# coop-columb/two-tower-amazon-recommender

Hardware: AMD Instinct MI355X
Metric: user-item pairs/sec (train step) + embedding-gather HBM GB/s, 1/2/4/8 MI355X (higher is better)
Workload: dtype f32; 1 GPU; cfg3: 5000000 users x 10000000 items, emb_dim 128, towers 128->256->128, batch 8192, in-batch sampled softmax T=0.1, sgd lr 1e-3, ids U; global_batch=8192, parallelism=single GPU

## Files before the change

### two_tower_amazon_recommender_amd/csrc/score.hip

```cpp
#include "common.h"

namespace {

using tt::f32x4;
using tt::f32x16;
typedef __bf16 bf16x4 __attribute__((ext_vector_type(4)));
typedef __bf16 bf16x8 __attribute__((ext_vector_type(8)));
typedef short s16x4 __attribute__((ext_vector_type(4)));

constexpr float kLog2e = 1.44269504088896340736f;
constexpr float kLn2 = 0.69314718055994530942f;
constexpr float kNegBig = -1.0e30f;

enum { MODE_FWD = 0, MODE_BWD = 1, MODE_FUSED = 2, MODE_RANK = 3, MODE_FUSED_S = 4, MODE_BWD_S = 5 };
constexpr float kRescaleThr = 8.0f;

struct ScoreArgs {
  const float* R;
  const float* K;
  int64_t n_r, n_c;
  int64_t diag;
  float c1;
  const float* a_r;
  const float* s_r;
  const float* a_c;
  const float* s_c;
  const int64_t* id_r;
  const int64_t* id_c;
  int nsplit;
  int64_t c_per_split;
  float* part_m;
  float* part_l;
  float* pos2;
  float* slab;
  const float* h_r;
  const float* h_c;
  const int64_t* pos_idx;
  int32_t* part_cnt;
  float* S;
  int64_t ldS;
};

template <int D, int PREC>
struct Geo {
  static constexpr int LS = D + 4;
  static constexpr int NG = D / 8;
  static constexpr int NB = D / 32;
  static constexpr int KS = D / 16;
  static constexpr int HALF_B = 32 * 256;
  static constexpr int PIECE_B = (D / 128) * HALF_B;
  static constexpr int TILE_F = PREC == 0 ? 32 * LS : 3 * PIECE_B / 4;
  static constexpr int BUF_F = TILE_F + 160;
  static constexpr int LDS_BYTES = 2 * BUF_F * 4;
};

struct Bf3 {
  __bf16 hi, mid, lo;
};
__device__ __forceinline__ Bf3 split3(float x) {
  Bf3 o;
  o.hi = (__bf16)x;
  const float r1 = x - (float)o.hi;
  o.mid = (__bf16)r1;
  o.lo = (__bf16)(r1 - (float)o.mid);
  return o;
}

__device__ __forceinline__ int img_off(int row, int ch) { return 256 * row + 16 * (ch ^ (((row & 3) << 2) | ((row >> 2) & 3))); }

constexpr int kBwdSWaves = 2;
constexpr int kSPrefetch = 2;
#ifndef TT_LOOP_LAMBDA
#define TT_LOOP_LAMBDA 0
#endif
constexpr int kTilesPerBarrier = 2;
constexpr int kTilesPerBarrierBwdS = kTilesPerBarrier;
template <int D, int MODE, int PREC>
constexpr int tiles_per_barrier() {
  if (PREC == 0 && D <= 128 && MODE == MODE_BWD_S) return kTilesPerBarrierBwdS;
  return (PREC == 0 && D <= 128 && (MODE == MODE_BWD || MODE == MODE_FUSED || MODE == MODE_FUSED_S))
             ? kTilesPerBarrier : 1;
}

template <int D, int MODE, int PREC>
constexpr bool split_d() {
  return PREC == 1 && D == 256 && (MODE == MODE_BWD || MODE == MODE_FUSED || MODE == MODE_FUSED_S);
}
template <int D, int MODE, bool HAS_IDS, bool HAS_HN, int PREC>
constexpr int rf_lds_groups() {
  if (PREC == 0 && D == 256 && (MODE == MODE_FUSED || MODE == MODE_FUSED_S) && (HAS_IDS || HAS_HN))
    return (HAS_IDS && HAS_HN) ? 10 : (HAS_HN ? 8 : 5);
  if (PREC == 0 && D == 128 && MODE == MODE_BWD && HAS_IDS && HAS_HN) return 2;
  return 0;
}
template <int D, int MODE, int PREC, int WAVES>
constexpr int rows_per_wg() { return (split_d<D, MODE, PREC>() ? WAVES / 2 : WAVES) * 32; }

template <int D, int MODE, bool HAS_IDS, bool HAS_HN, int WAVES, int PREC>
__global__ __launch_bounds__(WAVES * 64, (WAVES == 8 ? 2 : (D <= 128 ? ((MODE == MODE_BWD_S && PREC == 0) ? kBwdSWaves : 2) : 1))) void score_kernel(ScoreArgs p) {
  constexpr bool IS_FUSED = MODE == MODE_FUSED || MODE == MODE_FUSED_S;
  constexpr bool IS_BWD = MODE == MODE_BWD || MODE == MODE_BWD_S;
  constexpr bool FROM_S = MODE == MODE_BWD_S, TO_S = MODE == MODE_FUSED_S;
  using G_ = Geo<D, PREC>;
  constexpr int LS = G_::LS, NG = G_::NG, NB = G_::NB, TILE_F = G_::TILE_F, BUF_F = G_::BUF_F;
  constexpr int HALF_B = G_::HALF_B, PIECE_B = G_::PIECE_B;
  constexpr bool SPLIT = split_d<D, MODE, PREC>();
  constexpr int KS = SPLIT ? G_::KS / 2 : G_::KS;
  constexpr int NBW = SPLIT ? NB / 2 : NB;
  static_assert(PREC == 0 || D % 128 == 0, "bf16x3: dim 128 / 256 only (whole [32][128] bf16 images)");
  constexpr int ROW4 = D / 4;
  constexpr int THREADS = WAVES * 64;
  constexpr int NV = (32 * ROW4 + THREADS - 1) / THREADS;
  extern __shared__ __attribute__((aligned(16))) float smem[];

  const int tid = threadIdx.x;
  const int lane = tid & 63;
  const int wave = tid >> 6;
  const int h = lane >> 5;
  const int ln = lane & 31;

  const int split = __builtin_amdgcn_readfirstlane((int)(blockIdx.x % (unsigned)p.nsplit));
  const int64_t rblk = __builtin_amdgcn_readfirstlane((int)(blockIdx.x / (unsigned)p.nsplit));
  const int hw = SPLIT ? (wave & 1) : 0;
// ... 473 lines not shown
      if constexpr (IS_BWD || IS_FUSED) {
        if constexpr (PREC == 0) { if (t + TPB < ntiles) load_tile(t + TPB); }
        if constexpr (FROM_S) { if (t + 1 < ntiles) load_S(t + 1, xs); }
        gemm2(T, coef);
      }
      if (t + TPB < ntiles) store_tile((t + TPB) % NBUF);
      if ((t % TPB) == TPB - 1) __syncthreads();
    };
    for (int t = 0; t < ntiles; t += 2) {
      tile_step(t);
      if (t + 1 < ntiles) tile_step(t + 1);
    }
#else
    for (int t = 0; t < ntiles; ++t) {
      if constexpr (MODE == MODE_FWD || MODE == MODE_RANK || PREC == 1) { if (t + 1 < ntiles) load_tile(t + 1); }
      const float* T = smem + (t % NBUF) * BUF_F;
      f32x16 X;
      if constexpr (FROM_S) X = xs; else X = gemm1(T);
      if constexpr (SPLIT) exchange(X);
      if constexpr (TO_S) store_S(t, X);
      float coef[16];
      epilogue(T, t, X, coef);
      if constexpr (IS_BWD || IS_FUSED) {
        if constexpr (PREC == 0) { if (t + TPB < ntiles) load_tile(t + TPB); }
        if constexpr (FROM_S) { if (t + 1 < ntiles) load_S(t + 1, xs); }
        gemm2(T, coef);
      }
      if (t + TPB < ntiles) store_tile((t + TPB) % NBUF);
      if ((t % TPB) == TPB - 1) __syncthreads();
    }
#endif
  }

  if constexpr (IS_FUSED) {
    const float L = run_l + __shfl_xor(run_l, 32);
    if (r_ok && hw == 0) {
      if (h == 0) {
        p.part_m[(int64_t)split * p.n_r + r] = run_m;
        p.part_l[(int64_t)split * p.n_r + r] = L;
      }
      if (have_pos) p.pos2[r] = pos;
    }
  }
  if constexpr (MODE == MODE_RANK) {
    const int total = cnt + __shfl_xor(cnt, 32);
    if (r_ok && h == 0) p.part_cnt[(int64_t)split * p.n_r + r] = total;
  } else if constexpr (MODE == MODE_FWD) {
    const float om = __shfl_xor(run_m, 32);
    const float ol = __shfl_xor(run_l, 32);
    const float M = fmaxf(run_m, om);
    const float L = run_l * __builtin_amdgcn_exp2f(run_m - M) + ol * __builtin_amdgcn_exp2f(om - M);
    if (r_ok) {
      if (h == 0) {
        p.part_m[(int64_t)split * p.n_r + r] = M;
        p.part_l[(int64_t)split * p.n_r + r] = L;
      }
      if (have_pos) p.pos2[r] = pos;
    }
  } else {
    if (r_ok) {
      float* out = p.slab + ((int64_t)split * p.n_r + r) * D + 128 * hw;
      if constexpr (PREC == 1) {
#pragma unroll
        for (int b = 0; b < NBW; ++b)
#pragma unroll
          for (int g = 0; g < 4; ++g)
            *reinterpret_cast<f32x4*>(out + 32 * b + 8 * g + 4 * h) = f32x4{G[b][4 * g], G[b][4 * g + 1], G[b][4 * g + 2], G[b][4 * g + 3]};
      } else
#pragma unroll
      for (int reg = 0; reg < 16; ++reg) {
        const int i = tt::acc_row(reg, 0) + 4 * h;
        if constexpr (NB == 8) {
          *reinterpret_cast<f32x4*>(out + 8 * i) = f32x4{G[0][reg], G[1][reg], G[2][reg], G[3][reg]};
          *reinterpret_cast<f32x4*>(out + 8 * i + 4) = f32x4{G[4][reg], G[5][reg], G[6][reg], G[7][reg]};
        } else if constexpr (NB == 4) {
          *reinterpret_cast<f32x4*>(out + 4 * i) = f32x4{G[0][reg], G[1][reg], G[2][reg], G[3][reg]};
        } else if constexpr (NB == 2) {
          *reinterpret_cast<float2*>(out + 2 * i) = float2{G[0][reg], G[1][reg]};
        } else {
          out[i] = G[0][reg];
        }
      }
    }
  }
}


__global__ __launch_bounds__(256) void prob_bias_kernel(const float* __restrict__ prob, float* __restrict__ out, int64_t n) {
  const int64_t i = (int64_t)blockIdx.x * 256 + threadIdx.x;
  if (i < n) out[i] = -__log2f(fminf(fmaxf(prob[i], 1e-6f), 1.0f));
}

__global__ __launch_bounds__(256) void bwd_prep_kernel(const float* __restrict__ lse, const float* __restrict__ w,
                                                       float* __restrict__ a, float* __restrict__ s, int64_t n,
                                                       float scale) {
  const int64_t i = (int64_t)blockIdx.x * 256 + threadIdx.x;
  if (i < n) {
    a[i] = -lse[i] * kLog2e;
    s[i] = (w != nullptr ? w[i] : 1.0f) * scale;
  }
}

__global__ __launch_bounds__(256) void fwd_combine_kernel(const float* __restrict__ part_m, const float* __restrict__ part_l,
                                                          const float* __restrict__ pos2, const float* __restrict__ w,
                                                          int64_t n_r, int nsplit, float* __restrict__ lse,
                                                          float* __restrict__ per_row) {
  const int64_t r = (int64_t)blockIdx.x * 256 + threadIdx.x;
  if (r >= n_r) return;
  float M = kNegBig;
  for (int s = 0; s < nsplit; ++s) M = fmaxf(M, part_m[(int64_t)s * n_r + r]);
  float L = 0.f;
  for (int s = 0; s < nsplit; ++s)
    L += part_l[(int64_t)s * n_r + r] * __builtin_amdgcn_exp2f(part_m[(int64_t)s * n_r + r] - M);
  const float lse2 = M + __log2f(L);
  lse[r] = lse2 * kLn2;
  per_row[r] = (lse2 - pos2[r]) * kLn2 * (w != nullptr ? w[r] : 1.0f);
}

__global__ __launch_bounds__(256) void fused_combine_kernel(const float* __restrict__ part_m, const float* __restrict__ part_l,
                                                            const float* __restrict__ pos2, const float* __restrict__ w,
                                                            const f32x4* __restrict__ slab, const f32x4* __restrict__ cpos,
                                                            int64_t n_r, int d4, int lpr_log2, int nsplit, float scale,
                                                            float* __restrict__ lse, float* __restrict__ per_row,
                                                            float* __restrict__ aq, float* __restrict__ sq,
                                                            f32x4* __restrict__ dq) {
  const int rpb = 256 >> lpr_log2;
  const int64_t row = (int64_t)blockIdx.x * rpb + (threadIdx.x >> lpr_log2);
  const int lane = threadIdx.x & ((1 << lpr_log2) - 1);
  if (row >= n_r) return;
  constexpr int U = 8;
  const int c = lane < d4 ? lane : d4 - 1;
  const int last = nsplit - 1;
  f32x4 v0[U];
  const f32x4 cp = cpos[row * d4 + c];
#pragma unroll
  for (int u = 0; u < U; ++u) v0[u] = slab[((int64_t)(u < last ? u : last) * n_r + row) * d4 + c];
  const float p2 = pos2[row];
  const float wr = (w != nullptr ? w[row] : 1.0f);
  float pm0[U];
  float M = kNegBig;
  for (int s0 = 0; s0 < nsplit; s0 += U) {
    float pm[U];
#pragma unroll
    for (int u = 0; u < U; ++u) pm[u] = part_m[(int64_t)(s0 + u < last ? s0 + u : last) * n_r + row];
#pragma unroll
    for (int u = 0; u < U; ++u) {
      M = fmaxf(M, pm[u]);
      if (s0 == 0) pm0[u] = pm[u];
    }
  }
  float L = 0.f;
  for (int s0 = 0; s0 < nsplit; s0 += U) {
    float pm[U], pl[U];
#pragma unroll
    for (int u = 0; u < U; ++u) {
      const int64_t o = (int64_t)(s0 + u < last ? s0 + u : last) * n_r + row;
      pm[u] = part_m[o];
      pl[u] = part_l[o];
    }
#pragma unroll
    for (int u = 0; u < U; ++u)
      if (s0 + u < nsplit) L += pl[u] * __builtin_amdgcn_exp2f(pm[u] - M);
  }
  const float lse2 = M + __log2f(L);
  const float sr = wr * scale;
  if (lane == 0) {
// ... 68 lines not shown
  __shared__ int sh_remaining, sh_valid;
  const int tid = threadIdx.x;
  const int64_t row = blockIdx.x;
  const int64_t pos = row + diag;
  const float* srow = S + row * nc;
  const int64_t idpos = ids != nullptr ? ids[pos] : 0;
  auto valid = [&](int64_t j) { return j != pos && !(ids != nullptr && ids[j] == idpos); };
  auto keyof = [&](int64_t j) { return f2key(__builtin_fmaf(srow[j], c1, bias2 != nullptr ? bias2[j] : 0.f)); };
  if (tid == 0) { sh_prefix = 0; sh_mask = 0; sh_remaining = k; sh_valid = 0; sh_lower = 0; }
  __syncthreads();
  int nv = 0;
  for (int64_t j = tid; j < nc; j += 256) nv += valid(j) ? 1 : 0;
  atomicAdd(&sh_valid, nv);
  __syncthreads();
  if (k >= sh_valid) {
    if (tid == 0) thr[row] = -3.0e38f;
    return;
  }
  for (int pass = 0; pass < 4; ++pass) {
    const int shift = 24 - 8 * pass;
    hist[tid] = 0;
    __syncthreads();
    const uint32_t prefix = sh_prefix, mask = sh_mask;
    for (int64_t j = tid; j < nc; j += 256) {
      if (!valid(j)) continue;
      const uint32_t key = keyof(j);
      if ((key & mask) == prefix) atomicAdd(&hist[(key >> shift) & 255u], 1);
    }
    __syncthreads();
    if (tid == 0) {
      int cum = 0, rem = sh_remaining;
      for (int b = 255; b >= 0; --b) {
        if (cum + hist[b] >= rem) {
          sh_prefix = prefix | ((uint32_t)b << shift);
          sh_mask = mask | (255u << shift);
          sh_remaining = rem - cum;
          break;
        }
        cum += hist[b];
      }
    }
    __syncthreads();
  }
  const uint32_t key_k = sh_prefix;
  uint32_t lower = 0;
  for (int64_t j = tid; j < nc; j += 256) {
    if (!valid(j)) continue;
    const uint32_t key = keyof(j);
    if (key < key_k && key > lower) lower = key;
  }
  atomicMax(&sh_lower, lower);
  __syncthreads();
  if (tid == 0) {
    const float vk = key2f(key_k);
    const float vn = sh_lower != 0 ? key2f(sh_lower) : vk - 1.0f;
    thr[row] = 0.5f * vk + 0.5f * vn;
  }
}

__global__ __launch_bounds__(256) void hn_shift_kernel(const float* __restrict__ thr, const float* __restrict__ aq,
                                                       float* __restrict__ hq, int64_t n) {
  const int64_t i = (int64_t)blockIdx.x * 256 + threadIdx.x;
  if (i < n) hq[i] = thr[i] + aq[i];
}

__global__ __launch_bounds__(1024) void sum_rows_kernel(const float* __restrict__ per_row, int64_t n, float* __restrict__ loss) {
  __shared__ float red[1024];
  float acc = 0.f;
  for (int64_t r = threadIdx.x; r < n; r += 1024) acc += per_row[r];
  red[threadIdx.x] = acc;
  __syncthreads();
  for (int s = 512; s > 0; s >>= 1) {
    if ((int)threadIdx.x < s) red[threadIdx.x] += red[threadIdx.x + s];
    __syncthreads();
  }
  if (threadIdx.x == 0) loss[0] = red[0];
}

__global__ __launch_bounds__(256) void reduce_slabs_kernel(const f32x4* __restrict__ slab, f32x4* __restrict__ out,
                                                           int64_t n4, int nsplit, const float* __restrict__ per_row,
                                                           int64_t n_rows, float* __restrict__ loss) {
  if (per_row != nullptr && blockIdx.x == gridDim.x - 1) {
    __shared__ float red[256];
    const int t = threadIdx.x;
    float a[4] = {0.f, 0.f, 0.f, 0.f};
    for (int64_t r0 = t; r0 < n_rows; r0 += 8 * 1024) {
      float v[8][4];
#pragma unroll
      for (int i = 0; i < 8; ++i)
#pragma unroll
        for (int j = 0; j < 4; ++j) {
          const int64_t r = r0 + 1024 * i + 256 * j;
          v[i][j] = r < n_rows ? per_row[r] : 0.f;
        }
#pragma unroll
      for (int i = 0; i < 8; ++i)
#pragma unroll
        for (int j = 0; j < 4; ++j)
          if (r0 + 1024 * i + 256 * j < n_rows) a[j] += v[i][j];
    }
    red[t] = (a[0] + a[2]) + (a[1] + a[3]);
    __syncthreads();
    for (int s2 = 128; s2 > 0; s2 >>= 1) {
      if (t < s2) red[t] += red[t + s2];
      __syncthreads();
    }
    if (t == 0) loss[0] = red[0];
    return;
  }
  const int64_t nblk = per_row != nullptr ? gridDim.x - 1 : gridDim.x;
  const int64_t stride = nblk * 256;
  for (int64_t i = (int64_t)blockIdx.x * 256 + threadIdx.x; i < n4; i += stride) {
    f32x4 a = slab[i];
    for (int s = 1; s < nsplit; ++s) a += slab[(int64_t)s * n4 + i];
    out[i] = a;
  }
}


constexpr int kScoreWaves = 4;
constexpr int kScoreWgs = 512;
constexpr int kBwdSWgs = 512;
int choose_nsplit_pow2(int64_t n_r, int64_t n_c, int target_wgs = kScoreWgs) {
  const int64_t nrb = (n_r + 32 * kScoreWaves - 1) / (32 * kScoreWaves);
  int ns = 1;
  while (nrb * ns < target_wgs && (int64_t)ns * 2 * 64 <= n_c && ns < 64) ns *= 2;
  return ns;
}

int choose_nsplit(int64_t n_r, int64_t n_c, int rows_per_wg = 32 * kScoreWaves, int slots = kScoreWgs) {
  const int64_t nrb = (n_r + rows_per_wg - 1) / rows_per_wg;
  int best = 1;
  double best_cost = 0.0;
  for (int ns = 1; ns <= 64; ++ns) {
    if (ns > 1 && (int64_t)ns * 64 > n_c) break;
    const int64_t rounds = (nrb * ns + slots - 1) / slots;
    const double cost = (double)rounds / ns * (1.0 + 0.005 * ns);
    if (ns == 1 || cost < best_cost - 1e-12) { best = ns; best_cost = cost; }
  }
  return best;
}

int64_t align_up(int64_t x, int64_t a) { return (x + a - 1) / a * a; }

struct WsLayout {
  int ns_q, ns_c;
  int ns_cs;
  int64_t off_bias, off_aq, off_sq, off_hq, off_pm, off_pl, off_pos, off_slab, off_S, total_no_S, total;
};

WsLayout ws_layout(int64_t nq, int64_t nc, int32_t dim) {
  WsLayout w{};
  if (dim <= 128) {
    w.ns_q = choose_nsplit(nq, nc);
    w.ns_c = choose_nsplit(nc, nq);
    w.ns_cs = choose_nsplit(nc, nq, 256, 256);
  } else {
    w.ns_q = choose_nsplit_pow2(nq, nc);
    w.ns_c = choose_nsplit_pow2(nc, nq);
    w.ns_cs = choose_nsplit_pow2(nc, nq, kBwdSWgs);
  }
  int64_t o = 0;
  w.off_bias = o; o = align_up(o + nc * 4, 256);
  w.off_aq = o;   o = align_up(o + nq * 4, 256);
  w.off_sq = o;   o = align_up(o + nq * 4, 256);
  w.off_hq = o;   o = align_up(o + nq * 4, 256);
  w.off_pm = o;   o = align_up(o + (int64_t)w.ns_q * nq * 4, 256);
  w.off_pl = o;   o = align_up(o + (int64_t)w.ns_q * nq * 4, 256);
  w.off_pos = o;  o = align_up(o + nq * 4, 256);
  w.off_slab = o;
  const int64_t slab_q = (int64_t)w.ns_q * nq * dim * 4, slab_c = (int64_t)(w.ns_c > w.ns_cs ? w.ns_c : w.ns_cs) * nc * dim * 4;
  o = align_up(o + (slab_q > slab_c ? slab_q : slab_c), 256);
  w.total_no_S = o;
  w.off_S = o;
  o = align_up(o + ((nq + 31) / 32) * ((nc + 31) / 32) * 4096, 256);
  w.total = o;
  return w;
}

constexpr int kBwdSWgWaves = 8;
constexpr int kFusedSWgWaves = 4;
template <int D, int MODE, int PREC = 0>
constexpr int waves_for() {
  return (PREC == 1 && D == 128) ? 8 : (PREC == 1 ? 4 : ((MODE == MODE_BWD_S && D <= 128) ? kBwdSWgWaves
                                                         : ((MODE == MODE_FUSED_S && D <= 128) ? kFusedSWgWaves : kScoreWaves)));
}

template <int D, int MODE, int PREC = 0>
int launch_score(const ScoreArgs& a_in, bool has_ids, hipStream_t stream) {
  constexpr int W = waves_for<D, MODE, PREC>();
  constexpr int RPW = rows_per_wg<D, MODE, PREC, W>();
  const int64_t nrb = (a_in.n_r + RPW - 1) / RPW;
  const int64_t blocks = nrb * a_in.nsplit;
  const int lds_base = Geo<D, PREC>::LDS_BYTES * tiles_per_barrier<D, MODE, PREC>() +
                  ((PREC == 1 && W == 8) ? W * Geo<D, PREC>::KS * 64 * 16 : 0) +
                  (split_d<D, MODE, PREC>() ? W * 4096 : 0);
  const bool has_hn = (a_in.h_r != nullptr) || (a_in.h_c != nullptr);
  const ScoreArgs& a = a_in;
  auto go = [&](auto kern, int rfl_groups = 0) -> int {
    const int lds = lds_base + W * rfl_groups * 64 * 16;
    if (lds > 64 * 1024) {
      if (hipFuncSetAttribute(reinterpret_cast<const void*>(kern), hipFuncAttributeMaxDynamicSharedMemorySize, lds) != hipSuccess)
        return tt::fail(TT_ERR_LAUNCH, "hipFuncSetAttribute(LDS %d) failed", lds);
    }
    constexpr const char* tag = MODE == MODE_FWD ? "score_fwd" : ((MODE == MODE_BWD || MODE == MODE_BWD_S) ? "score_bwd"
                                : ((MODE == MODE_FUSED || MODE == MODE_FUSED_S) ? "score_fused" : "score_rank"));
    tt::launch(tag, kern, dim3((unsigned)blocks), dim3(W * 64), (unsigned)lds, stream, a);
    return tt::check_launch(tag);
  };
  if (has_ids && has_hn) return go(score_kernel<D, MODE, true, true, W, PREC>, rf_lds_groups<D, MODE, true, true, PREC>());
  if (has_ids) return go(score_kernel<D, MODE, true, false, W, PREC>, rf_lds_groups<D, MODE, true, false, PREC>());
  if (has_hn) return go(score_kernel<D, MODE, false, true, W, PREC>, rf_lds_groups<D, MODE, false, true, PREC>());
  return go(score_kernel<D, MODE, false, false, W, PREC>);
}

template <int MODE>
int dispatch_score_bx3(int32_t dim, const ScoreArgs& a, bool has_ids, hipStream_t stream) {
  switch (dim) {
    case 128: return launch_score<128, MODE, 1>(a, has_ids, stream);
    case 256: return launch_score<256, MODE, 1>(a, has_ids, stream);
    default: return tt::fail(TT_ERR_UNSUPPORTED, "retrieval (bf16x3): dim %d not in {128,256}", dim);
  }
}

template <int MODE>
int dispatch_score(int32_t dim, const ScoreArgs& a, bool has_ids, hipStream_t stream) {
  switch (dim) {
    case 32: return launch_score<32, MODE>(a, has_ids, stream);
    case 64: return launch_score<64, MODE>(a, has_ids, stream);
    case 128: return launch_score<128, MODE>(a, has_ids, stream);
    case 256: return launch_score<256, MODE>(a, has_ids, stream);
    default: return tt::fail(TT_ERR_UNSUPPORTED, "retrieval: dim %d not in {32,64,128,256}", dim);
  }
}

int check_common(const char* fn, const float* q, const float* c, int64_t nq, int64_t nc, int32_t dim,
                 int64_t diag_offset, const void* ws, int64_t ws_bytes, bool need_S = false) {
  TT_REQUIRE(q && c && ws, "%s: null pointer", fn);
  TT_REQUIRE(nq > 0 && nc > 0, "%s: nq and nc must be positive", fn);
  TT_REQUIRE(diag_offset >= 0 && nq + diag_offset <= nc, "%s: need 0 <= diag_offset and nq + diag_offset <= nc", fn);
  TT_REQUIRE(dim == 32 || dim == 64 || dim == 128 || dim == 256, "%s: dim %d not in {32,64,128,256}", fn, dim);
  TT_REQUIRE(tt::aligned16(q) && tt::aligned16(c), "%s: q/c must be 16-byte aligned", fn);
  TT_REQUIRE((reinterpret_cast<uintptr_t>(ws) & 255u) == 0, "%s: workspace must be 256-byte aligned", fn);
  const WsLayout wl = ws_layout(nq, nc, dim);
  const int64_t need = need_S ? wl.total : wl.total_no_S;
  if (ws_bytes < need)
    return tt::fail(TT_ERR_WORKSPACE, "%s: workspace %lld < %lld bytes", fn, (long long)ws_bytes, (long long)need);
  return TT_OK;
}

}

extern "C" int32_t tt_retrieval_num_splits(int64_t nq, int64_t nc, int32_t dim, int32_t pass) {
  if (nq <= 0 || nc <= 0 || dim <= 0 || pass < 0 || pass > 2) return 0;
  const WsLayout w = ws_layout(nq, nc, dim);
  return pass == 0 ? w.ns_q : (pass == 1 ? w.ns_c : w.ns_cs);
}

extern "C" int64_t tt_retrieval_workspace_bytes(int64_t nq, int64_t nc, int32_t dim) {
  if (nq <= 0 || nc <= 0 || dim <= 0) return 0;
  return ws_layout(nq, nc, dim).total;
}

extern "C" int64_t tt_retrieval_fwd_workspace_bytes(int64_t nq, int64_t nc, int32_t dim) {
  if (nq <= 0 || nc <= 0 || dim <= 0) return 0;
  return ws_layout(nq, nc, dim).total_no_S;
}

extern "C" int64_t tt_retrieval_rank_workspace_bytes(int64_t nq, int64_t nc, int32_t dim) {
  if (nq <= 0 || nc <= 0 || dim <= 0) return 0;
  return ws_layout(nq, nc, dim).off_pl;
}

static int retrieval_fwd(int prec, const float* q, const float* c, int64_t nq, int64_t nc, int32_t dim,
                         int64_t diag_offset, float inv_temperature, const float* sample_weight,
                         const float* cand_prob, const int64_t* cand_ids, const float* hard_thr,
                         void* workspace, int64_t workspace_bytes, float* lse, float* per_row, float* loss,
                         tt_stream_t stream_) {
  int rc = check_common("tt_retrieval_fwd_f32", q, c, nq, nc, dim, diag_offset, workspace, workspace_bytes);
  if (rc != TT_OK) return rc;
  TT_REQUIRE(lse && per_row && loss, "tt_retrieval_fwd_f32: null output pointer");
  hipStream_t stream = tt::as_stream(stream_);
  const WsLayout w = ws_layout(nq, nc, dim);
  char* ws = static_cast<char*>(workspace);
  float* bias = reinterpret_cast<float*>(ws + w.off_bias);
  if (cand_prob != nullptr) {
    hipLaunchKernelGGL(prob_bias_kernel, dim3((unsigned)((nc + 255) / 256)), dim3(256), 0, stream, cand_prob, bias, nc);
    if ((rc = tt::check_launch("prob_bias")) != TT_OK) return rc;
  }
  ScoreArgs a{};
  a.R = q; a.K = c; a.n_r = nq; a.n_c = nc; a.diag = diag_offset;
  a.c1 = kLog2e * inv_temperature;
  a.a_c = cand_prob != nullptr ? bias : nullptr;
  a.id_r = cand_ids != nullptr ? cand_ids + diag_offset : nullptr;
  a.id_c = cand_ids;
  a.h_r = hard_thr;
// ... 90 lines not shown
    a.id_c = cand_ids != nullptr ? cand_ids + diag_offset : nullptr;
    a.nsplit = w.ns_c;
    a.c_per_split = align_up((nq + a.nsplit - 1) / a.nsplit, 32);
    a.slab = slab;
    if ((rc = dispatch_score<MODE_BWD>(dim, a, cand_ids != nullptr, stream)) != TT_OK) return rc;
    const int64_t n4 = nc * dim / 4;
    const int64_t blocks = (n4 + 255) / 256 < 2048 ? (n4 + 255) / 256 : 2048;
    tt::launch("score_aux", reduce_slabs_kernel, dim3((unsigned)blocks), dim3(256), 0, stream,
               reinterpret_cast<const f32x4*>(slab), reinterpret_cast<f32x4*>(dc), n4, a.nsplit, (const float*)nullptr, (int64_t)0, (float*)nullptr);
    if ((rc = tt::check_launch("reduce_slabs(dc)")) != TT_OK) return rc;
  }
  return TT_OK;
}

static int retrieval_fwd_bwd(int prec, const float* q, const float* c, int64_t nq, int64_t nc, int32_t dim,
                             int64_t diag_offset, float inv_temperature, const float* sample_weight,
                             const float* cand_prob, const int64_t* cand_ids, const float* hard_thr,
                             float grad_scale, void* workspace, int64_t workspace_bytes, float* lse,
                             float* per_row, float* loss, float* dq, float* dc, tt_stream_t stream_) {
  int rc = check_common("tt_retrieval_fwd_bwd_f32", q, c, nq, nc, dim, diag_offset, workspace, workspace_bytes, true);
  if (rc != TT_OK) return rc;
  TT_REQUIRE(lse && per_row && loss && dq && dc, "tt_retrieval_fwd_bwd_f32: null output pointer");
  TT_REQUIRE(tt::aligned16(dq) && tt::aligned16(dc), "tt_retrieval_fwd_bwd_f32: dq/dc must be 16-byte aligned");
  hipStream_t stream = tt::as_stream(stream_);
  const WsLayout w = ws_layout(nq, nc, dim);
  char* ws = static_cast<char*>(workspace);
  float* bias = reinterpret_cast<float*>(ws + w.off_bias);
  float* aq = reinterpret_cast<float*>(ws + w.off_aq);
  float* sq = reinterpret_cast<float*>(ws + w.off_sq);
  float* slab = reinterpret_cast<float*>(ws + w.off_slab);
  float* smat = reinterpret_cast<float*>(ws + w.off_S);
  if (cand_prob != nullptr) {
    hipLaunchKernelGGL(prob_bias_kernel, dim3((unsigned)((nc + 255) / 256)), dim3(256), 0, stream, cand_prob, bias, nc);
    if ((rc = tt::check_launch("prob_bias")) != TT_OK) return rc;
  }
  const float* biasp = cand_prob != nullptr ? bias : nullptr;
  {
    ScoreArgs a{};
    a.R = q; a.K = c; a.n_r = nq; a.n_c = nc; a.diag = diag_offset;
    a.c1 = kLog2e * inv_temperature;
    a.a_c = biasp;
    a.h_r = hard_thr;
    a.S = smat; a.ldS = (nq + 31) / 32;
    a.id_r = cand_ids != nullptr ? cand_ids + diag_offset : nullptr;
    a.id_c = cand_ids;
    a.nsplit = w.ns_q;
    a.c_per_split = align_up((nc + a.nsplit - 1) / a.nsplit, 32);
    a.part_m = reinterpret_cast<float*>(ws + w.off_pm);
    a.part_l = reinterpret_cast<float*>(ws + w.off_pl);
    a.pos2 = reinterpret_cast<float*>(ws + w.off_pos);
    a.slab = slab;
    rc = prec == 1 ? dispatch_score_bx3<MODE_FUSED_S>(dim, a, cand_ids != nullptr, stream)
                   : dispatch_score<MODE_FUSED_S>(dim, a, cand_ids != nullptr, stream);
    if (rc != TT_OK) return rc;
    {
      int lpr_log2 = 3;
      while ((1 << lpr_log2) < dim / 4) ++lpr_log2;
      const int rpb = 256 >> lpr_log2;
      tt::launch("score_aux", fused_combine_kernel, dim3((unsigned)((nq + rpb - 1) / rpb)), dim3(256), 0, stream, a.part_m, a.part_l, a.pos2,
                         sample_weight, reinterpret_cast<const f32x4*>(slab),
                         reinterpret_cast<const f32x4*>(c + diag_offset * dim), nq, dim / 4, lpr_log2, a.nsplit,
                         inv_temperature * grad_scale, lse, per_row, aq, sq, reinterpret_cast<f32x4*>(dq));
      if ((rc = tt::check_launch("fused_combine")) != TT_OK) return rc;
    }
  }
  float* hq = nullptr;
  if (hard_thr != nullptr) {
    hq = reinterpret_cast<float*>(ws + w.off_hq);
    hipLaunchKernelGGL(hn_shift_kernel, dim3((unsigned)((nq + 255) / 256)), dim3(256), 0, stream, hard_thr, aq, hq, nq);
    if ((rc = tt::check_launch("hn_shift")) != TT_OK) return rc;
  }
  {
    ScoreArgs a{};
    a.R = c; a.K = q; a.n_r = nc; a.n_c = nq; a.diag = -diag_offset;
    a.c1 = kLog2e * inv_temperature;
    a.a_r = biasp; a.s_r = nullptr; a.a_c = aq; a.s_c = sq;
    a.h_c = hq;
    a.id_r = cand_ids;
    a.id_c = cand_ids != nullptr ? cand_ids + diag_offset : nullptr;
    a.nsplit = w.ns_cs;
    a.c_per_split = align_up((nq + a.nsplit - 1) / a.nsplit, 32);
    a.slab = slab;
    a.S = smat; a.ldS = (nq + 31) / 32;
    rc = prec == 1 ? dispatch_score_bx3<MODE_BWD_S>(dim, a, cand_ids != nullptr, stream)
                   : dispatch_score<MODE_BWD_S>(dim, a, cand_ids != nullptr, stream);
    if (rc != TT_OK) return rc;
    const int64_t n4 = nc * dim / 4;
    const int64_t blocks = (n4 + 255) / 256 < 2048 ? (n4 + 255) / 256 : 2048;
    tt::launch("score_aux", reduce_slabs_kernel, dim3((unsigned)blocks + 1), dim3(256), 0, stream,
                       reinterpret_cast<const f32x4*>(slab), reinterpret_cast<f32x4*>(dc), n4, a.nsplit, per_row, nq, loss);
    if ((rc = tt::check_launch("reduce_slabs(dc)")) != TT_OK) return rc;
  }
  return TT_OK;
}

extern "C" int tt_retrieval_fwd_bwd_f32(const float* q, const float* c, int64_t nq, int64_t nc, int32_t dim,
                                        int64_t diag_offset, float inv_temperature, const float* sample_weight,
                                        const float* cand_prob, const int64_t* cand_ids, const float* hard_thr,
                                        float grad_scale, void* workspace, int64_t workspace_bytes, float* lse,
                                        float* per_row, float* loss, float* dq, float* dc, tt_stream_t stream) {
  return retrieval_fwd_bwd(0, q, c, nq, nc, dim, diag_offset, inv_temperature, sample_weight, cand_prob, cand_ids, hard_thr,
                           grad_scale, workspace, workspace_bytes, lse, per_row, loss, dq, dc, stream);
}

extern "C" int tt_retrieval_fwd_bwd_bf16x3_f32(const float* q, const float* c, int64_t nq, int64_t nc, int32_t dim,
                                               int64_t diag_offset, float inv_temperature, const float* sample_weight,
                                               const float* cand_prob, const int64_t* cand_ids, const float* hard_thr,
                                               float grad_scale, void* workspace, int64_t workspace_bytes, float* lse,
                                               float* per_row, float* loss, float* dq, float* dc, tt_stream_t stream) {
  if (dim != 128 && dim != 256) return tt::fail(TT_ERR_UNSUPPORTED, "tt_retrieval_fwd_bwd_bf16x3_f32: dim %d not in {128,256}", dim);
  return retrieval_fwd_bwd(1, q, c, nq, nc, dim, diag_offset, inv_temperature, sample_weight, cand_prob, cand_ids, hard_thr,
                           grad_scale, workspace, workspace_bytes, lse, per_row, loss, dq, dc, stream);
}

static int retrieval_rank(int prec, const float* q, const float* c, int64_t nq, int64_t nc, int32_t dim,
                          float inv_temperature, const float* cand_prob, const int64_t* pos_index,
                          void* workspace, int64_t workspace_bytes, int32_t* rank, tt_stream_t stream_) {
  int rc;
  TT_REQUIRE(q && c && workspace && pos_index && rank, "tt_retrieval_rank_f32: null pointer");
  TT_REQUIRE(nq > 0 && nc > 0, "tt_retrieval_rank_f32: nq and nc must be positive");
  TT_REQUIRE(dim == 32 || dim == 64 || dim == 128 || dim == 256, "tt_retrieval_rank_f32: dim %d not in {32,64,128,256}", dim);
  TT_REQUIRE(tt::aligned16(q) && tt::aligned16(c), "tt_retrieval_rank_f32: q/c must be 16-byte aligned");
  TT_REQUIRE((reinterpret_cast<uintptr_t>(workspace) & 255u) == 0, "tt_retrieval_rank_f32: workspace must be 256-byte aligned");
  const WsLayout w = ws_layout(nq, nc, dim);
  if (workspace_bytes < w.off_pl)
    return tt::fail(TT_ERR_WORKSPACE, "tt_retrieval_rank_f32: workspace %lld < %lld bytes", (long long)workspace_bytes,
                    (long long)w.off_pl);
  hipStream_t stream = tt::as_stream(stream_);
  char* ws = static_cast<char*>(workspace);
  float* bias = reinterpret_cast<float*>(ws + w.off_bias);
  float* thr = reinterpret_cast<float*>(ws + w.off_aq);
  int32_t* part_cnt = reinterpret_cast<int32_t*>(ws + w.off_pm);
  const float c1 = kLog2e * inv_temperature;
  if (cand_prob != nullptr) {
    hipLaunchKernelGGL(prob_bias_kernel, dim3((unsigned)((nc + 255) / 256)), dim3(256), 0, stream, cand_prob, bias, nc);
    if ((rc = tt::check_launch("prob_bias")) != TT_OK) return rc;
  }
  const float* biasp = cand_prob != nullptr ? bias : nullptr;
  hipLaunchKernelGGL(pos_logit_kernel, dim3((unsigned)((nq + 7) / 8)), dim3(256), 0, stream, reinterpret_cast<const f32x4*>(q),
                     reinterpret_cast<const f32x4*>(c), pos_index, biasp, nq, nc, dim / 4, c1, thr, (int64_t)0);
  if ((rc = tt::check_launch("pos_logit")) != TT_OK) return rc;
  ScoreArgs a{};
  a.R = q; a.K = c; a.n_r = nq; a.n_c = nc; a.diag = 0;
  a.c1 = c1;
  a.a_r = thr; a.a_c = biasp;
  a.pos_idx = pos_index;
  a.nsplit = w.ns_q;
  a.c_per_split = align_up((nc + a.nsplit - 1) / a.nsplit, 32);
  a.part_cnt = part_cnt;
  rc = prec == 1 ? dispatch_score_bx3<MODE_RANK>(dim, a, false, stream) : dispatch_score<MODE_RANK>(dim, a, false, stream);
  if (rc != TT_OK) return rc;
  hipLaunchKernelGGL(rank_combine_kernel, dim3((unsigned)((nq + 255) / 256)), dim3(256), 0, stream, part_cnt, nq, a.nsplit, rank);
  return tt::check_launch("rank_combine");
}

extern "C" int tt_retrieval_rank_f32(const float* q, const float* c, int64_t nq, int64_t nc, int32_t dim,
                                     float inv_temperature, const float* cand_prob, const int64_t* pos_index,
                                     void* workspace, int64_t workspace_bytes, int32_t* rank, tt_stream_t stream) {
  return retrieval_rank(0, q, c, nq, nc, dim, inv_temperature, cand_prob, pos_index, workspace, workspace_bytes, rank, stream);
}

extern "C" int tt_retrieval_rank_bf16x3_f32(const float* q, const float* c, int64_t nq, int64_t nc, int32_t dim,
                                            float inv_temperature, const float* cand_prob, const int64_t* pos_index,
                                            void* workspace, int64_t workspace_bytes, int32_t* rank, tt_stream_t stream) {
  if (dim != 128 && dim != 256) return tt::fail(TT_ERR_UNSUPPORTED, "tt_retrieval_rank_bf16x3_f32: dim %d not in {128,256}", dim);
  return retrieval_rank(1, q, c, nq, nc, dim, inv_temperature, cand_prob, pos_index, workspace, workspace_bytes, rank, stream);
// ... 69 lines not shown
```

Baseline: 14.71 million pairs/s.

## Add streaming dc backward kernel with in-LDS split reduction and fused loss sum

Result: no change. 14.85 million pairs/s (median of 6 runs) (+1.0%).

```diff
diff --git a/two_tower_amazon_recommender_amd/csrc/score.hip b/two_tower_amazon_recommender_amd/csrc/score.hip
--- a/two_tower_amazon_recommender_amd/csrc/score.hip
+++ b/two_tower_amazon_recommender_amd/csrc/score.hip
@@ -39,6 +39,10 @@
   int32_t* part_cnt;
   float* S;
   int64_t ldS;
+  float* out;
+  const float* loss_rows;
+  int64_t n_loss_rows;
+  float* loss;
 };
 
 template <int D, int PREC>
@@ -678,6 +682,202 @@
         }
       }
     }
+  }
+}
+
+__device__ __forceinline__ void sum_rows_256(const float* __restrict__ per_row, int64_t n_rows, float* __restrict__ loss, float* red) {
+  const int t = threadIdx.x;
+  if (t < 256) {
+    float a[4] = {0.f, 0.f, 0.f, 0.f};
+    for (int64_t r0 = t; r0 < n_rows; r0 += 8 * 1024) {
+      float v[8][4];
+#pragma unroll
+      for (int i = 0; i < 8; ++i)
+#pragma unroll
+        for (int j = 0; j < 4; ++j) {
+          const int64_t r = r0 + 1024 * i + 256 * j;
+          v[i][j] = r < n_rows ? per_row[r] : 0.f;
+        }
+#pragma unroll
+      for (int i = 0; i < 8; ++i)
+#pragma unroll
+        for (int j = 0; j < 4; ++j)
+          if (r0 + 1024 * i + 256 * j < n_rows) a[j] += v[i][j];
+    }
+    red[t] = (a[0] + a[2]) + (a[1] + a[3]);
+  }
+  __syncthreads();
+#pragma unroll
+  for (int s2 = 128; s2 > 0; s2 >>= 1) {
+    if (t < s2) red[t] += red[t + s2];
+    __syncthreads();
+  }
+  if (t == 0) loss[0] = red[0];
+}
+
+constexpr int kDcRing = 8;
+template <int D, bool HAS_IDS, bool HAS_HN>
+__global__ __launch_bounds__(512, 2) void dc_stream_kernel(ScoreArgs p) {
+  static_assert(D == 128, "one 16-byte load per lane and register step: dim 128");
+  constexpr int NB = D / 32;
+  constexpr int RING = HAS_IDS ? kDcRing / 2 : kDcRing;
+  extern __shared__ __attribute__((aligned(16))) float smem[];
+  if (blockIdx.x == gridDim.x - 1) {
+    sum_rows_256(p.loss_rows, p.n_loss_rows, p.loss, smem);
+    return;
+  }
+  const int lane = threadIdx.x & 63;
+  const int wave = __builtin_amdgcn_readfirstlane((int)(threadIdx.x >> 6));
+  const int h = lane >> 5;
+  const int ln = lane & 31;
+  const int split = wave;
+  const int64_t r0w = (int64_t)__builtin_amdgcn_readfirstlane((int)blockIdx.x) * 32;
+  const int64_t r = r0w + ln;
+  const bool r_ok = r < p.n_r;
+  const int64_t rl = r_ok ? r : p.n_r - 1;
+  const bool tail_wave = r0w + 32 > p.n_r;
+  const int64_t c_begin = (int64_t)split * p.c_per_split;
+  int64_t c_end = c_begin + p.c_per_split;
+  if (c_end > p.n_c) c_end = p.n_c;
+  const int ntiles = __builtin_amdgcn_readfirstlane((split < p.nsplit && c_end > c_begin) ? (int)((c_end - c_begin + 31) >> 5) : 0);
+  const int ncols = (int)(c_end - c_begin);
+
+  const float ar = p.a_r != nullptr ? p.a_r[rl] : 0.f;
+  const float sr = p.s_r != nullptr ? p.s_r[rl] : 1.f;
+  const float hr = (HAS_HN && p.h_r != nullptr) ? p.h_r[rl] : -3.0e38f;
+  int64_t idr = 0;
+  if constexpr (HAS_IDS) idr = p.id_r[rl];
+  const int64_t cpos = r + p.diag;
+
+  f32x16 G[NB];
+#pragma unroll
+  for (int b = 0; b < NB; ++b)
+#pragma unroll
+    for (int i = 0; i < 16; ++i) G[b][i] = 0.f;
+
+  if (ntiles > 0) {
+    auto tile_of = [&](int t) { return t < ntiles ? t : ntiles - 1; };
+    auto lim_of = [&](int tc) { const int l = ncols - 1 - 32 * tc; return l < 31 ? l : 31; };
+    const float* kq = p.K + c_begin * D;
+    auto load_k = [&](int t, int reg) -> f32x4 {
+      const int tc = tile_of(t), lim = lim_of(tc);
+      const int row = tt::acc_row(reg, 0) + 4 * h;
+      return *reinterpret_cast<const f32x4*>(kq + (int64_t)tc * (32 * D) + (unsigned)((row < lim ? row : lim) * D + NB * ln));
+    };
+    const float* sblk = p.S + ((r0w >> 5) * p.ldS + (c_begin >> 5)) * 1024;
+    auto load_X = [&](int t, f32x16& X) {
+      const float* blk = sblk + (int64_t)tile_of(t) * 1024 + (unsigned)(4 * h * 32 + ln);
+#pragma unroll
+      for (int reg = 0; reg < 16; ++reg) X[reg] = blk[tt::acc_row(reg, 0) * 32];
+    };
+    const float* acp = p.a_c + c_begin;
+    const float* scp = p.s_c + c_begin;
+    const float* hcp = HAS_HN ? p.h_c + c_begin : nullptr;
+    f32x4 n_a[4], n_s[4], n_h[4];
+    int64_t n_id[HAS_IDS ? 16 : 1];
+    auto load_vecs = [&](int t) {
+      const int tc = tile_of(t), lim = lim_of(tc);
+#pragma unroll
+      for (int g = 0; g < 4; ++g) {
+        const int e = 8 * g + 4 * h;
+        const unsigned o = (unsigned)(e < (lim & ~3) ? e : (lim & ~3));
+        n_a[g] = *reinterpret_cast<const f32x4*>(acp + 32 * tc + o);
+        n_s[g] = *reinterpret_cast<const f32x4*>(scp + 32 * tc + o);
+        if constexpr (HAS_HN) n_h[g] = *reinterpret_cast<const f32x4*>(hcp + 32 * tc + o);
+      }
+      if constexpr (HAS_IDS) {
+        const int64_t* idp = p.id_c + c_begin + 32 * tc;
+#pragma unroll
+        for (int reg = 0; reg < 16; ++reg) {
+          const int e = tt::acc_row(reg, 0) + 4 * h;
+          n_id[reg] = idp[(unsigned)(e < lim ? e : lim)];
+        }
+      }
+    };
+
+    f32x16 xs;
+    f32x4 kr[RING];
+    load_vecs(0);
+    __builtin_amdgcn_sched_barrier(0);
+    load_X(0, xs);
+    __builtin_amdgcn_sched_barrier(0);
+#pragma unroll
+    for (int i = 0; i < RING; ++i) kr[i] = load_k(0, i);
+    __builtin_amdgcn_sched_barrier(0);
+
+#pragma nounroll
+    for (int t = 0; t < ntiles; ++t) {
+      const int64_t c0 = c_begin + 32 * (int64_t)t;
+      const int nq_left = ncols - 32 * t;
+      float ac[16], sc[16], hth[16];
+#pragma unroll
+      for (int g = 0; g < 4; ++g)
+#pragma unroll
+        for (int i = 0; i < 4; ++i) {
+          ac[4 * g + i] = n_a[g][i];
+          sc[4 * g + i] = n_s[g][i];
+          if constexpr (HAS_HN) hth[4 * g + i] = fmaxf(n_h[g][i], hr);
+        }
+      const bool diag_tile = (c0 < r0w + p.diag + 32) && (c0 + 32 > r0w + p.diag);
+      int dloc = -100;
+      if (diag_tile) {
+        const int64_t dd = cpos - c0;
+        dloc = (dd >= 0 && dd < 32) ? (int)dd - 4 * h : -100;
+      }
+      bool dup[16];
+      if constexpr (HAS_IDS) {
+#pragma unroll
+        for (int reg = 0; reg < 16; ++reg) dup[reg] = (n_id[reg] == idr) && (tt::acc_row(reg, 0) != dloc);
+      }
+      float coef[16], tvs[16];
+#pragma unroll
+      for (int reg = 0; reg < 16; ++reg) tvs[reg] = __builtin_fmaf(xs[reg], p.c1, ac[reg]) + ar;
+#pragma unroll
+      for (int reg = 0; reg < 16; ++reg) {
+        const float w = sc[reg] * sr;
+        float tv = tvs[reg];
+        if constexpr (HAS_HN) tv = (tv < hth[reg] && tt::acc_row(reg, 0) != dloc) ? kNegBig : tv;
+        float e = __builtin_amdgcn_exp2f(tv) * w;
+        if constexpr (HAS_IDS) e = dup[reg] ? 0.f : e;
+        coef[reg] = e;
+      }
+      if (diag_tile) {
+#pragma unroll
+        for (int reg = 0; reg < 16; ++reg)
+          if (tt::acc_row(reg, 0) == dloc) coef[reg] -= sc[reg] * sr;
+      }
+      if (nq_left < 32 || tail_wave) {
+#pragma unroll
+        for (int reg = 0; reg < 16; ++reg)
+          coef[reg] = (r_ok && tt::acc_row(reg, 0) + 4 * h < nq_left) ? coef[reg] : 0.f;
+      }
+      load_vecs(t + 1);
+      load_X(t + 1, xs);
+#pragma unroll
+      for (int reg = 0; reg < 16; ++reg) {
+        const f32x4 kc = kr[reg % RING];
+        kr[reg % RING] = load_k(t + (reg + RING) / 16, (reg + RING) % 16);
+#pragma unroll
+        for (int b = 0; b < NB; ++b) G[b] = __builtin_amdgcn_mfma_f32_32x32x2f32(kc[b], coef[reg], G[b], 0, 0, 0);
+        __builtin_amdgcn_sched_barrier(0);
+      }
+    }
+  }
+
+  f32x4* part = reinterpret_cast<f32x4*>(smem);
+  if (split < p.nsplit) {
+#pragma unroll
+    for (int reg = 0; reg < 16; ++reg) {
+      const int i = tt::acc_row(reg, 0) + 4 * h;
+      part[split * 1024 + i * 32 + ln] = f32x4{G[0][reg], G[1][reg], G[2][reg], G[3][reg]};
+    }
+  }
+  __syncthreads();
+  for (int e = threadIdx.x; e < 1024; e += blockDim.x) {
+    f32x4 a = part[e];
+    for (int s = 1; s < p.nsplit; ++s) a += part[s * 1024 + e];
+    const int row = e & 31, i = e >> 5;
+    if (r0w + row < p.n_r) *reinterpret_cast<f32x4*>(p.out + (r0w + row) * D + 4 * i) = a;
   }
 }
 
@@ -912,30 +1112,7 @@
                                                            int64_t n_rows, float* __restrict__ loss) {
   if (per_row != nullptr && blockIdx.x == gridDim.x - 1) {
     __shared__ float red[256];
-    const int t = threadIdx.x;
-    float a[4] = {0.f, 0.f, 0.f, 0.f};
-    for (int64_t r0 = t; r0 < n_rows; r0 += 8 * 1024) {
-      float v[8][4];
-#pragma unroll
-      for (int i = 0; i < 8; ++i)
-#pragma unroll
-        for (int j = 0; j < 4; ++j) {
-          const int64_t r = r0 + 1024 * i + 256 * j;
-          v[i][j] = r < n_rows ? per_row[r] : 0.f;
-        }
-#pragma unroll
-      for (int i = 0; i < 8; ++i)
-#pragma unroll
-        for (int j = 0; j < 4; ++j)
-          if (r0 + 1024 * i + 256 * j < n_rows) a[j] += v[i][j];
-    }
-    red[t] = (a[0] + a[2]) + (a[1] + a[3]);
-    __syncthreads();
-    for (int s2 = 128; s2 > 0; s2 >>= 1) {
-      if (t < s2) red[t] += red[t + s2];
-      __syncthreads();
-    }
-    if (t == 0) loss[0] = red[0];
+    sum_rows_256(per_row, n_rows, loss, red);
     return;
   }
   const int64_t nblk = per_row != nullptr ? gridDim.x - 1 : gridDim.x;
@@ -1042,6 +1219,32 @@
   if (has_ids) return go(score_kernel<D, MODE, true, false, W, PREC>, rf_lds_groups<D, MODE, true, false, PREC>());
   if (has_hn) return go(score_kernel<D, MODE, false, true, W, PREC>, rf_lds_groups<D, MODE, false, true, PREC>());
   return go(score_kernel<D, MODE, false, false, W, PREC>);
+}
+
+constexpr int kDcMaxRanges = 8;
+constexpr int64_t kDcMaxQBytes = 4 << 20;
+template <int D>
+int launch_dc_stream(const ScoreArgs& a, bool has_ids, hipStream_t stream) {
+  if (a.a_c == nullptr || a.s_c == nullptr || a.S == nullptr || a.out == nullptr || a.loss_rows == nullptr || a.loss == nullptr ||
+      a.nsplit < 1 || a.nsplit > kDcMaxRanges)
+    return tt::fail(TT_ERR_INVALID_ARG, "dc_stream: bad arguments");
+  const int64_t blocks = (a.n_r + 31) / 32 + 1;
+  const int waves = a.nsplit < 4 ? 4 : a.nsplit;
+  const int lds = a.nsplit * 16384;
+  if (a.h_r != nullptr && a.h_c == nullptr) return tt::fail(TT_ERR_INVALID_ARG, "dc_stream: hard-negative thresholds come per query (h_c)");
+  const bool has_hn = a.h_c != nullptr;
+  auto go = [&](auto kern) -> int {
+    if (lds > 64 * 1024) {
+      if (hipFuncSetAttribute(reinterpret_cast<const void*>(kern), hipFuncAttributeMaxDynamicSharedMemorySize, lds) != hipSuccess)
+        return tt::fail(TT_ERR_LAUNCH, "hipFuncSetAttribute(LDS %d) failed", lds);
+    }
+    tt::launch("score_bwd", kern, dim3((unsigned)blocks), dim3(waves * 64), (unsigned)lds, stream, a);
+    return tt::check_launch("score_bwd");
+  };
+  if (has_ids && has_hn) return go(dc_stream_kernel<D, true, true>);
+  if (has_ids) return go(dc_stream_kernel<D, true, false>);
+  if (has_hn) return go(dc_stream_kernel<D, false, true>);
+  return go(dc_stream_kernel<D, false, false>);
 }
 
 template <int MODE>
@@ -1298,6 +1501,10 @@
     a.c_per_split = align_up((nq + a.nsplit - 1) / a.nsplit, 32);
     a.slab = slab;
     a.S = smat; a.ldS = (nq + 31) / 32;
+    if (prec == 0 && dim == 128 && a.nsplit <= kDcMaxRanges && nq * dim * 4 <= kDcMaxQBytes) {
+      a.out = dc; a.loss_rows = per_row; a.n_loss_rows = nq; a.loss = loss;
+      return launch_dc_stream<128>(a, cand_ids != nullptr, stream);
+    }
     rc = prec == 1 ? dispatch_score_bx3<MODE_BWD_S>(dim, a, cand_ids != nullptr, stream)
                    : dispatch_score<MODE_BWD_S>(dim, a, cand_ids != nullptr, stream);
     if (rc != TT_OK) return rc;
```
